# rust-cv/cv

Measured on AMD Instinct MI355X. Metric: frames/sec AKAZE detect+describe+BF-Hamming-match, 1080p, higher is better.
Workload: dtype f32; 1 GPU; BASELINE configs[1]: batch of 256 synthetic 1920x1080 frames per GPU (ONE panning camera over a single seeded world canvas, 4 px right / 2 px down per frame, +-2 sensor noise per frame — not SURVEY 8d's per-frame seeds: consecutive frames must overlap for the match to mean something), Akaze::default() detect+describe, + symmetric better-by-24 BF Hamming match of consecutive frames; micro_batch=256, parallelism=frame-sharded x1

## Files before the change

### cv_amd/_lib.py

```python
import ctypes as C
import os

import numpy as np

_HERE = os.path.dirname(os.path.abspath(__file__))
LIB_PATH = os.path.join(_HERE, "lib", "libakz.so")


class AkzError(RuntimeError):
    def __init__(self, status, what=""):
        self.status = status
        msg = lib().akz_strerror(status).decode()
        hip = lib().akz_last_hip_error()
        if status == -5 and hip:
            msg += f" (hip {hip}: {lib().akz_last_hip_error_string().decode()})"
        super().__init__(f"{what}: {msg}" if what else msg)


class Config(C.Structure):
    _fields_ = [
        ("maximum_features", C.c_uint64),
        ("num_sublevels", C.c_uint32),
        ("max_octave_evolution", C.c_uint32),
        ("base_scale_offset", C.c_double),
# ... 6 lines not shown
        ("descriptor_pattern_size", C.c_uint64),
    ]


class Options(C.Structure):
    _fields_ = [
        ("struct_size", C.c_uint32), ("flags", C.c_uint32), ("fed_block", C.c_uint32),
        ("sup_capacity", C.c_uint32), ("max_candidates", C.c_uint32), ("desc_tile_shift", C.c_uint32),
        ("stream_waves", C.c_uint32), ("stream_min_waves", C.c_uint32), ("arith", C.c_uint32), ("cu_ss", C.c_uint32),
        ("cu_kp", C.c_uint32), ("resident_min_frames", C.c_uint32), ("reserved", C.c_uint32 * 4),
    ]


OPT_KEEP_ALL, OPT_NO_FRAME_PAIRS, OPT_SERIAL_SUPPRESSION, OPT_NO_PIPELINE = 1, 2, 4, 8
OPT_STREAM_PRIORITY, OPT_CONTRAST_EXACT, OPT_CONTRAST_FORCE_ODD, OPT_TILE_KERNELS, OPT_SERIAL_DET, OPT_SPLIT_FRONT_FED, OPT_EQUAL_PRIORITY, OPT_NO_RESIDENT_LEVELS = 16, 32, 64, 128, 256, 512, 1024, 2048
HM_OPT_NO_FP4, HM_OPT_NO_MFMA, HM_OPT_STREAM_PRIORITY, HM_OPT_NO_LDS_DMA = 1, 2, 4, 8
FMT_U8, FMT_F32, FMT_U16 = 0, 1, 2
ARITH_REDUCE_PAIRWISE, ARITH_FMA, ARITH_HALF_SEQUENTIAL = 1, 2, 4


BOOL_OPTIONS = ("keep_all", "frame_pairs", "parallel_suppression", "pipeline", "stream_priority", "stream_kernels",
                "det_side_stream", "fuse_front_fed", "resident_levels")


def make_options(keep_all=False, frame_pairs=True, parallel_suppression=True, pipeline=True, stream_priority=True,
                 contrast="fine", fed_block=0, sup_capacity=0, max_candidates=0, desc_tile_shift=0, stream_kernels=True,
                 stream_waves=0, stream_min_waves=0, det_side_stream=True, fuse_front_fed=True, arith=0, cu_ss=0, cu_kp=0,
                 resident_levels=True, resident_min_frames=0):
    o = Options()
    o.struct_size = C.sizeof(Options)
    o.flags = ((OPT_KEEP_ALL if keep_all else 0) | (0 if frame_pairs else OPT_NO_FRAME_PAIRS)
               | (0 if parallel_suppression else OPT_SERIAL_SUPPRESSION) | (0 if pipeline else OPT_NO_PIPELINE)
               | (0 if stream_priority else OPT_EQUAL_PRIORITY) | (0 if stream_kernels else OPT_TILE_KERNELS)
               | (0 if det_side_stream else OPT_SERIAL_DET) | (0 if fuse_front_fed else OPT_SPLIT_FRONT_FED)
               | (0 if resident_levels else OPT_NO_RESIDENT_LEVELS)
               | {"fine": 0, "exact": OPT_CONTRAST_EXACT, "force_odd": OPT_CONTRAST_FORCE_ODD}[contrast])
    o.fed_block, o.sup_capacity, o.max_candidates, o.desc_tile_shift = fed_block, sup_capacity, max_candidates, desc_tile_shift
    o.stream_waves, o.stream_min_waves = stream_waves, stream_min_waves
    o.arith = arith
    o.cu_ss, o.cu_kp = cu_ss, cu_kp
    o.resident_min_frames = resident_min_frames
    return o


class ArrsacParams(C.Structure):
    _fields_ = [("struct_size", C.c_uint32), ("n_hypotheses", C.c_uint32), ("block_size", C.c_uint32),
                ("init_blocks", C.c_uint32), ("max_candidates", C.c_uint32), ("flags", C.c_uint32),
                ("threshold", C.c_double), ("sprt_delta", C.c_double), ("sprt_ratio", C.c_double), ("seed", C.c_uint64),
                ("estimations_per_block", C.c_uint32), ("reserved", C.c_uint32)]

# ... 210 lines not shown
```

### cv_amd/csrc/akz_api.hip

```cpp
#include <math.h>
#include <stdio.h>

#include <new>

#include "akz_ctx.h"

thread_local int g_akz_last_hip = 0;

extern "C" const char* akz_version(void) { return "cv_amd-akz 0.5 (gfx950)"; }
extern "C" uint32_t akz_abi_version(void) { return AKZ_ABI_VERSION; }

extern "C" const char* akz_strerror(int32_t s)
{
    switch (s) {
    case AKZ_OK: return "ok";
    case AKZ_E_INVALID: return "invalid argument or unsupported configuration";
    case AKZ_E_NO_DEVICE: return "no usable HIP device";
    case AKZ_E_OOM: return "out of device memory";
    case AKZ_E_CAPACITY: return "output buffer too small";
    case AKZ_E_HIP: return "HIP runtime error";
    case AKZ_E_TOO_LARGE: return "image or batch larger than the context was created for";
    case AKZ_E_INTERNAL: return "device-side overflow of an internal work list (create the context with a larger max_keypoints / akz_options.max_candidates)";
    case AKZ_E_COMM: return "RCCL call failed or librccl.so.1 could not be loaded (akz_comm_last_error_string())";
    default: return "unknown status";
// ... 117 lines not shown
{
    return akz_guard([&]() -> int32_t {
        if (!cfg || !out || max_w < 3 || max_h < 3 || max_batch < 1 || max_w > 65535 || max_h > 65535) return AKZ_E_INVALID;
        if ((size_t)max_w * (size_t)max_h > kAkzMaxPixels) return AKZ_E_TOO_LARGE;
        AKZ_TRY(validate_config(cfg));
        akz_options o;
        memset(&o, 0, sizeof(o));
        if (opts) {
            if (opts->struct_size < 2 * sizeof(uint32_t) || opts->struct_size > 4096) return AKZ_E_INVALID;
            memcpy(&o, opts, opts->struct_size < sizeof(o) ? opts->struct_size : sizeof(o));
            for (uint32_t i = (uint32_t)sizeof(o); i < opts->struct_size; ++i)
                if (reinterpret_cast<const unsigned char*>(opts)[i]) return AKZ_E_INVALID;
            if (o.cu_ss > 32 || o.cu_kp > 32) return AKZ_E_INVALID;
            for (uint32_t r : o.reserved)
                if (r) return AKZ_E_INVALID;
            if (o.flags & ~((AKZ_OPT_NO_RESIDENT_LEVELS << 1) - 1u)) return AKZ_E_INVALID;
            if (o.fed_block > 8 || (o.desc_tile_shift != 0 && (o.desc_tile_shift < 2 || o.desc_tile_shift > 9))) return AKZ_E_INVALID;
            if (o.arith > 7u) return AKZ_E_INVALID;
            if (o.sup_capacity > (1u << 24) || o.max_candidates > kAkzMaxKeypoints || o.stream_waves > (1u << 24) ||
                o.stream_min_waves > (1u << 24))
                return AKZ_E_INVALID;
        }
        {
            AkzPlan probe;
            akz_build_plan(*cfg, max_w, max_h, &probe);
            if ((int)probe.levels.size() > kAkzMaxLevels) return AKZ_E_INVALID;
        }
        int ndev = 0;
        hipError_t e = hipGetDeviceCount(&ndev);
        if (e != hipSuccess || ndev <= 0 || device < 0 || device >= ndev) {
            g_akz_last_hip = (int)e;
// ... 11 lines not shown
        c->max_w = max_w;
        c->max_h = max_h;
        c->max_batch = max_batch;
        c->max_kp = max_keypoints ? max_keypoints : 16384u;
        if (c->max_kp > kAkzMaxKeypoints) c->max_kp = kAkzMaxKeypoints;
        c->max_cand = o.max_candidates ? o.max_candidates : c->max_kp;
        if (c->max_cand > kAkzMaxKeypoints) c->max_cand = kAkzMaxKeypoints;
        c->sup_cap = o.sup_capacity ? o.sup_capacity : 4u * c->max_kp;
        c->sup_parallel = !(o.flags & AKZ_OPT_SERIAL_SUPPRESSION);
        c->keep_all = (o.flags & AKZ_OPT_KEEP_ALL) != 0;
        c->front_pair = !(o.flags & AKZ_OPT_NO_FRAME_PAIRS);
        c->stream_kernels = !(o.flags & AKZ_OPT_TILE_KERNELS);
        c->det_side_stream = !(o.flags & AKZ_OPT_SERIAL_DET);
        c->fuse_front_fed = !(o.flags & AKZ_OPT_SPLIT_FRONT_FED);
        c->resident_levels = !(o.flags & AKZ_OPT_NO_RESIDENT_LEVELS);
        c->resident_min_frames = (int)o.resident_min_frames;
        c->arith = (int)o.arith;
        if (o.stream_waves) c->det_stream_waves = (int)o.stream_waves;
        if (o.stream_min_waves) c->stream_min_waves = (size_t)o.stream_min_waves;
        c->contrast_fine = !(o.flags & AKZ_OPT_CONTRAST_EXACT);
        c->contrast_force_odd = (o.flags & AKZ_OPT_CONTRAST_FORCE_ODD) != 0;
        c->nsets = (o.flags & AKZ_OPT_NO_PIPELINE) ? 1 : 2;
        if (o.fed_block) c->fed_block = (int)o.fed_block;
        if (o.desc_tile_shift) c->desc_tile_shift = (int)o.desc_tile_shift;
        int32_t st = AKZ_OK;
        int prio_lo = 0, prio_hi = 0;
        hipDeviceGetStreamPriorityRange(&prio_lo, &prio_hi);
        const bool use_prio = !(o.flags & AKZ_OPT_EQUAL_PRIORITY);
        if (o.cu_ss) {
            if (akz_stream_on_cus(&c->stream, 0, (int)o.cu_ss) != hipSuccess) st = AKZ_E_HIP;
// ... 710 lines not shown
```

### cv_amd/csrc/akz_ctx.h

```cpp
#pragma once
#include <utility>

#include <hip/hip_ext.h>

#include "akz_common.h"

typedef akz_keypoint DevKp;

struct AkzTimer {
    std::vector<std::pair<hipEvent_t, hipEvent_t>> pending;
    std::vector<hipEvent_t> pool;
    hipEvent_t cur_start = nullptr;
    double ms = 0.0;
    uint64_t launches = 0, units = 0, units2 = 0;
};

struct AkzSet {
    std::vector<float*> Lt, Lsm, Ldet, Lflow;
    std::vector<float2*> Lxy;
    float* tmp = nullptr;
    void* d_in = nullptr;
    unsigned long long* d_cmax = nullptr;
    uint32_t* d_hist = nullptr;
    uint32_t* d_npoints = nullptr;
// ... 55 lines not shown

    AkzPlan plan;
    int cur_w = 0, cur_h = 0, cur_n = 0;

    void* arena = nullptr;
    size_t arena_bytes = 0;
    AkzSet sets[2];
    int nsets = 2;
    int cur = 0;
    uint64_t calls = 0;
    hipStream_t stream_kp = nullptr;
    hipStream_t stream_det = nullptr;
    bool det_side_stream = true;
    bool fuse_front_fed = true;
    bool resident_levels = true;
    int resident_min_frames = 0;
    hipEvent_t ev_level[kAkzMaxLevels] = {};
    hipEvent_t ev_det_done = nullptr;
    bool sup_parallel = true;
    uint32_t sup_cap = 0;
    void* d_color = nullptr;
    size_t color_bytes = 0;
    hipEvent_t ev_ss_done[2] = {nullptr, nullptr};
    hipEvent_t ev_kp_done[2] = {nullptr, nullptr};
    bool kp_pending[2] = {false, false};
    hipEvent_t ev_input = nullptr;
    AkzSet& S() { return sets[cur]; }
    void* h_in = nullptr;
    size_t h_in_bytes = 0;
    void* h_out = nullptr;
// ... 55 lines not shown
```

### cv_amd/csrc/akz_scale_space.hip

```cpp
#include "akz_ctx.h"

#ifndef AKZ_ARITH
#define AKZ_ARITH 0
#endif
#define AKZ_SS_CAT2(a, b) a##b
#define AKZ_SS_CAT(a, b) AKZ_SS_CAT2(a, b)
#define AKZ_SS(name) AKZ_SS_CAT(name##_arith, AKZ_ARITH)

namespace {

constexpr bool kArithPairwise = (AKZ_ARITH & 1) != 0;
constexpr bool kArithFma = (AKZ_ARITH & 2) != 0;
constexpr bool kArithHalfSeq = (AKZ_ARITH & 4) != 0;

constexpr int kTW = 64;
constexpr int kTH = 32;
constexpr int kDTH = 12;

enum { EPI_BLUR = 0, EPI_FLOW = 1, EPI_CMAX = 2, EPI_CHIST = 3 };

__device__ __forceinline__ int clampi(int v, int lo, int hi) { return v < lo ? lo : (v > hi ? hi : v); }

__device__ __forceinline__ uint3 xcd_tile_linear(uint32_t orig, uint3 grid);
__device__ __forceinline__ uint3 xcd_tile(uint3 bid, uint3 grid)
// ... 1019 lines not shown
    float v = l0;
    if (x < w - 1) v = v + fed_flow(half_tau, c0, C[1], l0, L[1]);
    if (x > 0) v = v - fed_flow(half_tau, C[-1], c0, L[-1], l0);
    if (y < h - 1) v = v + fed_flow(half_tau, c0, C[w], l0, L[w]);
    if (y > 0) v = v - fed_flow(half_tau, C[-w], c0, L[-w], l0);
    dst[base] = v;
}

constexpr int kFedMaxBlock = 16;
struct FedTaus {
    float half_tau[kFedMaxBlock];
};

constexpr int fed_halo_patches(int T) { return (T + 3) / 4; }
constexpr int fed_tile_edge(int T) { return 64 - 8 * fed_halo_patches(T); }

__device__ __forceinline__ v2f fed_flow2(v2f ht, v2f ca, v2f cb, v2f a, v2f b) { return (ht * (ca + cb)) * (b - a); }

__device__ __forceinline__ void fed_steps(v2f (&L)[4][4], v2f (&C)[4][4], float4* __restrict__ s_top,
                                          float4* __restrict__ s_ct, float4* __restrict__ s_vd, const FedTaus& taus,
                                          int nsteps, int tid, int up, int dn, int x0, int y0, int w, int h)
{
    s_ct[tid * 2] = make_float4(C[0][0].x, C[0][0].y, C[0][1].x, C[0][1].y);
    s_ct[tid * 2 + 1] = make_float4(C[0][2].x, C[0][2].y, C[0][3].x, C[0][3].y);
    const bool z_right = x0 + 4 <= 0 || x0 + 4 >= w;
    bool z_below[4];
#pragma unroll
    for (int r = 0; r < 4; ++r) z_below[r] = y0 + r < 0 || y0 + r >= h - 1;
#pragma unroll 1
    for (int t = 0; t < nsteps; ++t) {
// ... 33 lines not shown
                for (int c = 0; c < 4; ++c) vu[c] = fed_flow2(htu, C[r - (r > 0)][c], C[r][c], L[r - (r > 0)][c], L[r][c]);
            } else {
                __syncthreads();
                const float4 a = s_vd[up * 2], b = s_vd[up * 2 + 1];
                vu[0] = (v2f){a.x, a.y}; vu[1] = (v2f){a.z, a.w}; vu[2] = (v2f){b.x, b.y}; vu[3] = (v2f){b.z, b.w};
            }
#pragma unroll
            for (int c = 0; c < 4; ++c) {
                L[r][c] = (((L[r][c] + hf[c + 1]) - hf[c]) + vd[c]) - vu[c];
                vd[c] = vu[c];
            }
        }
    }
}

__device__ __forceinline__ void fed_steps_sums(v2f (&L)[4][4], const v2f (&C)[4][4], float4* __restrict__ s_top,
                                               float4* __restrict__ s_ct, float4* __restrict__ s_vd, const FedTaus& taus,
                                               int nsteps, int tid, int up, int dn, int x0, int y0, int w, int h)
{
    s_ct[tid * 2] = make_float4(C[0][0].x, C[0][0].y, C[0][1].x, C[0][1].y);
    s_ct[tid * 2 + 1] = make_float4(C[0][2].x, C[0][2].y, C[0][3].x, C[0][3].y);
    v2f SH[4][4], SV[4][4];
#pragma unroll
    for (int r = 0; r < 4; ++r) {
        const v2f Cr = dpp_row<0x101>(C[r][0]);
#pragma unroll
        for (int c = 0; c < 3; ++c) SH[r][c] = C[r][c] + C[r][c + 1];
        SH[r][3] = C[r][3] + Cr;
    }
#pragma unroll
    for (int r = 0; r < 3; ++r)
#pragma unroll
        for (int c = 0; c < 4; ++c) SV[r][c] = C[r][c] + C[r + 1][c];
    __syncthreads();
    {
        const float4 c = s_ct[dn * 2], d = s_ct[dn * 2 + 1];
        SV[3][0] = C[3][0] + (v2f){c.x, c.y};
        SV[3][1] = C[3][1] + (v2f){c.z, c.w};
        SV[3][2] = C[3][2] + (v2f){d.x, d.y};
        SV[3][3] = C[3][3] + (v2f){d.z, d.w};
    }
    const bool z_right = x0 + 4 <= 0 || x0 + 4 >= w;
    bool z_below[4];
#pragma unroll
    for (int r = 0; r < 4; ++r) z_below[r] = y0 + r < 0 || y0 + r >= h - 1;
#pragma unroll 1
    for (int t = 0; t < nsteps; ++t) {
        const float htf = taus.half_tau[t];
        const v2f ht = splat(htf);
        s_top[tid * 2] = make_float4(L[0][0].x, L[0][0].y, L[0][1].x, L[0][1].y);
        s_top[tid * 2 + 1] = make_float4(L[0][2].x, L[0][2].y, L[0][3].x, L[0][3].y);
        __syncthreads();
        v2f vd[4];
        {
            const float4 a = s_top[dn * 2], b = s_top[dn * 2 + 1];
            const v2f Lb[4] = {(v2f){a.x, a.y}, (v2f){a.z, a.w}, (v2f){b.x, b.y}, (v2f){b.z, b.w}};
            const v2f ht3 = splat(z_below[3] ? 0.0f : htf);
#pragma unroll
            for (int cc = 0; cc < 4; ++cc) vd[cc] = (ht3 * SV[3][cc]) * (Lb[cc] - L[3][cc]);
            s_vd[tid * 2] = make_float4(vd[0].x, vd[0].y, vd[1].x, vd[1].y);
            s_vd[tid * 2 + 1] = make_float4(vd[2].x, vd[2].y, vd[3].x, vd[3].y);
        }
        const v2f htr = splat(z_right ? 0.0f : htf);
#pragma unroll
        for (int r = 3; r >= 0; --r) {
            const v2f Lr = dpp_row<0x101>(L[r][0]);
            v2f hf[5];
#pragma unroll
            for (int c = 1; c < 4; ++c) hf[c] = (ht * SH[r][c - 1]) * (L[r][c] - L[r][c - 1]);
            hf[4] = (htr * SH[r][3]) * (Lr - L[r][3]);
            hf[0] = dpp_row<0x111>(hf[4]);
            v2f vu[4];
            if (r > 0) {
                const v2f htu = splat(z_below[r > 0 ? r - 1 : 0] ? 0.0f : htf);
#pragma unroll
                for (int c = 0; c < 4; ++c) vu[c] = (htu * SV[r - (r > 0)][c]) * (L[r][c] - L[r - (r > 0)][c]);
            } else {
                __syncthreads();
                const float4 a = s_vd[up * 2], b = s_vd[up * 2 + 1];
                vu[0] = (v2f){a.x, a.y}; vu[1] = (v2f){a.z, a.w}; vu[2] = (v2f){b.x, b.y}; vu[3] = (v2f){b.z, b.w};
            }
#pragma unroll
            for (int c = 0; c < 4; ++c) {
                L[r][c] = (((L[r][c] + hf[c + 1]) - hf[c]) + vd[c]) - vu[c];
                vd[c] = vu[c];
            }
        }
    }
}

__device__ __forceinline__ void fed_store_patch(const v2f (&L)[4][4], float* __restrict__ dst, int fa, int fb, bool has_b,
                                                size_t fs, int w, int h, int x0, int y0)
{
    float* da = dst + (size_t)fa * fs;
    float* db = dst + (size_t)fb * fs;
// ... 101 lines not shown
                                                const float* __restrict__ srcb, int w, int wx0, int wy0, int tid)
{
    constexpr int NCH = kFFIn * (kFFInC / 4);
#pragma unroll
    for (int i = 0; i < ITEMS; ++i) {
        const int idx = tid + 256 * i;
        if (idx < NCH) {
            const int iy = idx / (kFFInC / 4), c4 = idx - iy * (kFFInC / 4);
            const uint32_t o = (uint32_t)((wy0 - 3 + iy) * w + (wx0 - 4 + 4 * c4)) << 2;
            ra[i] = *reinterpret_cast<const float4*>(at_bytes(srca, o));
            rb[i] = *reinterpret_cast<const float4*>(at_bytes(srcb, o));
        }
    }
}

template <int SG, int HP, bool RING, bool WRITE_FLOW>
__global__ __launch_bounds__(256, kFFWaves) void k_front_fed(const float* __restrict__ in, int w, int h, size_t fs, int n,
                                                      GaussTaps taps, OffK k, FedTaus taus, int nsteps,
                                                      float* __restrict__ out_lt, float* __restrict__ out_flow,
                                                      float2* __restrict__ out_xy, const float* __restrict__ invk,
                                                      int invk_off, float* __restrict__ half_out, size_t half_fs)
{
    __shared__ __attribute__((aligned(16))) v2f s_buf[kFFIn * kFFInC];
    static_assert((kFFW + 2) * kFFGS <= kFFIn * kFFInC, "blurred window fits in the input window's space");
    static_assert(3 * 256 * 2 * 2 <= kFFIn * kFFInC, "FED exchange buffers fit");
    constexpr int U = front_fed_tile(HP);
    const uint3 tile = xcd_tile(make_uint3(blockIdx.x, blockIdx.y, blockIdx.z), make_uint3(gridDim.x, gridDim.y, gridDim.z));
    const int tid = threadIdx.x, pc = tid & 15, pr = tid >> 4;
    const int fa = 2 * (int)tile.z;
    const bool has_b = fa + 1 < n;
    const int fb = has_b ? fa + 1 : fa;
    const int wx0 = (int)tile.x * U - 4 * HP, wy0 = (int)tile.y * U - 4 * HP;
    const float* srca = in + (size_t)fa * fs;
    const float* srcb = in + (size_t)fb * fs;
    {
        const bool inside = wx0 >= 4 && wx0 + kFFW + 4 <= w && wy0 >= 3 && wy0 + kFFW + 3 <= h;
        if (inside) {
            constexpr int NCH = kFFIn * (kFFInC / 4), ITEMS = (NCH + 255) / 256;
            float4 ra[ITEMS], rb[ITEMS];
            front_fed_fetch<ITEMS>(ra, rb, srca, srcb, w, wx0, wy0, tid);
            float4* d = reinterpret_cast<float4*>(s_buf);
#pragma unroll
            for (int i = 0; i < ITEMS; ++i) {
                const int idx = tid + 256 * i;
                if (idx < NCH) {
                    const int iy = idx / (kFFInC / 4), c4 = idx - iy * (kFFInC / 4);
                    d[ff_chunk<kFFInC / 2>(iy, 2 * c4)] = make_float4(ra[i].x, rb[i].x, ra[i].y, rb[i].y);
                    d[ff_chunk<kFFInC / 2>(iy, 2 * c4 + 1)] = make_float4(ra[i].z, rb[i].z, ra[i].w, rb[i].w);
                }
            }
        } else {
            constexpr int NE = kFFIn * kFFInC, BATCH = 8;
            for (int base = 0; base < NE; base += 256 * BATCH) {
                float ea[BATCH], eb[BATCH];
#pragma unroll
                for (int i = 0; i < BATCH; ++i) {
                    const int idx = base + tid + 256 * i;
                    ea[i] = eb[i] = 0.0f;
                    if (idx < NE) {
                        const int iy = idx / kFFInC, ix = idx - iy * kFFInC;
                        const int cx = clampi(wx0 - 4 + ix, 0, w - 1), cy = clampi(wy0 - 3 + iy, 0, h - 1);
                        const size_t o = (size_t)cy * w + cx;
                        ea[i] = srca[o];
                        eb[i] = srcb[o];
                    }
                }
#pragma unroll
                for (int i = 0; i < BATCH; ++i) {
                    const int idx = base + tid + 256 * i;
                    if (idx < NE) {
                        const int iy = idx / kFFInC, ix = idx - iy * kFFInC;
                        s_buf[ff_elem<kFFInC / 2>(iy, ix)] = (v2f){ea[i], eb[i]};
                    }
                }
            }
        }
    }
    __syncthreads();
    v2f g[4][4];
// ... 73 lines not shown
            }
        }
#pragma unroll
        for (int j = 0; j < 4; ++j)
#pragma unroll
            for (int o = 0; o < 4; ++o) {
                const v2f col[5] = {hb[j][o], hb[j + 1][o], hb[j + 2][o], hb[j + 3][o], hb[j + 4][o]};
                g[j][o] = lane4_dot_v<5>(col, taps.k);
            }
    }
    __syncthreads();
    v2f* s_g = s_buf;
    float4* g4 = reinterpret_cast<float4*>(s_buf);
#pragma unroll
    for (int j = 0; j < 4; ++j) {
        g4[ff_chunk<kFFGS / 2>(4 * pr + j + 1, 2 * pc + 1)] = make_float4(g[j][0].x, g[j][0].y, g[j][1].x, g[j][1].y);
        g4[ff_chunk<kFFGS / 2>(4 * pr + j + 1, 2 * pc + 2)] = make_float4(g[j][2].x, g[j][2].y, g[j][3].x, g[j][3].y);
    }
#pragma unroll
    for (int q = 0; q < 2; ++q)
        if (RING && tid + 256 * q < 4 * kFFW + 4) s_g[ff_elem<kFFGS / 2>(ring_y[q] + 1, ring_x[q] + 2)] = ring[q];
    __syncthreads();
    if (wx0 < 1 || wx0 + kFFW + 1 > w || wy0 < 1 || wy0 + kFFW + 1 > h) {
#pragma unroll
        for (int j = 0; j < 4; ++j)
#pragma unroll
            for (int o = 0; o < 4; ++o) {
                const int x = wx0 + 4 * pc + o, y = wy0 + 4 * pr + j;
                const int xc = clampi(x, 0, w - 1), yc = clampi(y, 0, h - 1);
                if (xc != x || yc != y) {
                    const int X = clampi(xc - wx0, -1, kFFW), Y = clampi(yc - wy0, -1, kFFW);
                    s_g[ff_elem<kFFGS / 2>(4 * pr + j + 1, 4 * pc + o + 2)] = s_g[ff_elem<kFFGS / 2>(Y + 1, X + 2)];
                }
            }
#pragma unroll
        for (int q = 0; q < 2; ++q)
            if (RING && tid + 256 * q < 4 * kFFW + 4) {
                const int x = wx0 + ring_x[q], y = wy0 + ring_y[q];
                const int xc = clampi(x, 0, w - 1), yc = clampi(y, 0, h - 1);
                if (xc != x || yc != y) {
                    const int X = clampi(xc - wx0, -1, kFFW), Y = clampi(yc - wy0, -1, kFFW);
                    s_g[ff_elem<kFFGS / 2>(ring_y[q] + 1, ring_x[q] + 2)] = s_g[ff_elem<kFFGS / 2>(Y + 1, X + 2)];
                }
            }
        __syncthreads();
    }
    const int x0 = wx0 + 4 * pc, y0 = wy0 + 4 * pr;
    const bool col_in = x0 >= 0 && x0 < w;
    const bool useful = pc >= HP && pc <= 15 - HP && pr >= HP && pr <= 15 - HP && col_in;
    v2f C[4][4];
    {
        const v2f inverse_k = (v2f){invk[(size_t)fa * 8 + invk_off], invk[(size_t)fb * 8 + invk_off]};
        v2f hx[3][4], hy[3][4];
#pragma unroll
        for (int r = 0; r < 6; ++r) {
            v2f v[8];
#pragma unroll
            for (int q = 0; q < 4; ++q) {
                const f4v t = lds_chunk(g4 + ff_chunk<kFFGS / 2>(4 * pr + r, 2 * pc + q));
                v[2 * q] = (v2f){t.x, t.y};
                v[2 * q + 1] = (v2f){t.z, t.w};
            }
            const int s = r % 3;
#pragma unroll
            for (int o = 0; o < 4; ++o) {
                hx[s][o] = v[o + 3] - v[o + 1];
                hy[s][o] = (splat(3.0f) * v[o + 1] + splat(10.0f) * v[o + 2]) + splat(3.0f) * v[o + 3];
            }
            if (r >= 2) {
                const int j = r - 2, sm = (r - 2) % 3, s0 = (r - 1) % 3, sp = r % 3;
                v2f den[4];
#pragma unroll
                for (int o = 0; o < 4; ++o) {
                    const v2f lx = (splat(3.0f) * hx[sm][o] + splat(10.0f) * hx[s0][o]) + splat(3.0f) * hx[sp][o];
// ... 6 lines not shown
#pragma unroll
                    for (int o = 0; o < 4; ++o) C[j][o] = splat(1.0f) / den[o];
                } else {
#pragma unroll
                    for (int o = 0; o < 4; ++o) C[j][o] = rcp_pair_finite(den[o]);
                }
            }
        }
    }
    if (WRITE_FLOW && useful) {
#pragma unroll
        for (int j = 0; j < 4; ++j) {
            const int y = y0 + j;
            if (y >= h) break;
            const uint32_t o = (uint32_t)(y * w + x0) << 2;
            *reinterpret_cast<float4*>(at_bytes(out_flow + (size_t)fa * fs, o)) = make_float4(C[j][0].x, C[j][1].x, C[j][2].x, C[j][3].x);
            if (has_b)
                *reinterpret_cast<float4*>(at_bytes(out_flow + (size_t)fb * fs, o)) = make_float4(C[j][0].y, C[j][1].y, C[j][2].y, C[j][3].y);
        }
    }
    if (useful) {
#pragma unroll
        for (int j = 0; j < 4; ++j) {
            const int y = y0 + j;
            if (y >= h) break;
            v2f m[12], z[12], p[12];
            const int Y = 4 * pr + j;
            constexpr int Q0 = (4 - SG) / 2, Q1 = (7 + SG) / 2;
#pragma unroll
            for (int q = Q0; q <= Q1; ++q) {
                const f4v a = lds_chunk(g4 + ff_chunk<kFFGS / 2>(Y - SG + 1, 2 * pc - 1 + q));
                const f4v b = lds_chunk(g4 + ff_chunk<kFFGS / 2>(Y + 1, 2 * pc - 1 + q));
                const f4v c = lds_chunk(g4 + ff_chunk<kFFGS / 2>(Y + SG + 1, 2 * pc - 1 + q));
                m[2 * q] = (v2f){a.x, a.y}; m[2 * q + 1] = (v2f){a.z, a.w};
                z[2 * q] = (v2f){b.x, b.y}; z[2 * q + 1] = (v2f){b.z, b.w};
                p[2 * q] = (v2f){c.x, c.y}; p[2 * q + 1] = (v2f){c.z, c.w};
            }
            v2f rx[4], ry[4];
#pragma unroll
            for (int o = 0; o < 4; ++o) {
                const v2f mm = m[4 + o - SG], m0 = m[4 + o], mp = m[4 + o + SG];
                const v2f zm = z[4 + o - SG], zp = z[4 + o + SG];
                const v2f pm = p[4 + o - SG], p0 = p[4 + o], pp = p[4 + o + SG];
                rx[o] = off_combine_sg<SG>(k, mp - mm, zp - zm, pp - pm);
                ry[o] = off_combine_sg<SG>(k, pm, p0, pp) - off_combine_sg<SG>(k, mm, m0, mp);
            }
            const uint32_t o = (uint32_t)(y * w + x0) << 3;
            {
                float4* xy = reinterpret_cast<float4*>(at_bytes(out_xy + (size_t)fa * fs, o));
                xy[0] = make_float4(rx[0].x, ry[0].x, rx[1].x, ry[1].x);
                xy[1] = make_float4(rx[2].x, ry[2].x, rx[3].x, ry[3].x);
            }
            if (has_b) {
                float4* xy = reinterpret_cast<float4*>(at_bytes(out_xy + (size_t)fb * fs, o));
                xy[0] = make_float4(rx[0].y, ry[0].y, rx[1].y, ry[1].y);
                xy[1] = make_float4(rx[2].y, ry[2].y, rx[3].y, ry[3].y);
            }
        }
    }
#pragma unroll
    for (int r = 0; r < 4; ++r) {
        const int y = y0 + r;
        const bool in_img = col_in && y >= 0 && y < h;
        if (!in_img) {
#pragma unroll
            for (int c = 0; c < 4; ++c) {
                L[r][c] = splat(0.0f);
                C[r][c] = splat(0.0f);
            }
        }
    }
    __syncthreads();
    float4* s_top = reinterpret_cast<float4*>(s_buf);
    float4* s_vd = s_top + 256 * 2;
    float4* s_ct = s_vd + 256 * 2;
    const int up = pr > 0 ? tid - 16 : tid, dn = pr < 15 ? tid + 16 : tid;
    fed_steps_sums(L, C, s_top, s_ct, s_vd, taus, nsteps, tid, up, dn, x0, y0, w, h);
    if (useful) {
        fed_store_patch(L, out_lt, fa, fb, has_b, fs, w, h, x0, y0);
        if (half_out) fed_store_half(L, half_out, fa, fb, has_b, half_fs, w, h, x0, y0);
    }
}

constexpr int kResMaxSteps = 64;
struct FedTausN {
    float half_tau[kResMaxSteps];
};
constexpr int kResLdsBytes = 160 * 1024 - 2048;
#ifndef AKZ_RES_R
#define AKZ_RES_R 6
#define AKZ_RES_WAVES 12
#endif

__device__ __forceinline__ int res_chunk(int rs, int row, int ci) { return row * rs + ((ci & 1) ? (rs >> 1) : 0) + (ci >> 1); }
__device__ __forceinline__ int res_elem(int rs, int row, int col) { return 2 * res_chunk(rs, row, col >> 1) + (col & 1); }
// ... 1212 lines not shown
                    int ngr = (left + fed_block - 1) / fed_block;
                    int g = (left + ngr - 1) / ngr;
                    groups.push_back(g);
                    left -= g;
                }
            const bool front_fed = c->fuse_front_fed && blocked && fused_front && !c->keep_all && !groups.empty() &&
                                   groups[0] <= (L.octave == 0 ? 4 : 8);
            if (front_fed) {
                const int ng = (int)groups.size();
                float* dst0 = ((ng - 1) % 2 == 0) ? bufA : bufB;
                FedTaus ft;
                for (int q = 0; q < kFedMaxBlock; ++q) ft.half_tau[q] = q < groups[0] ? 0.5f * (float)L.tau[q] : 0.0f;
                OffK kk = make_offk(L.deriv_sigma);
                const int t_ff = (L.octave == 0 ? AKZ_T_FRONT_FED_SG2 : AKZ_T_FRONT_FED_DEEP_SG2) + (int)L.deriv_sigma - 2;
                akz_timer_begin(c, t_ff, s);
#define AKZ_FF3(SGV, HPV, RGV, WFV)                                                                                  \
    AKZ_LAUNCH((k_front_fed<SGV, HPV, RGV, WFV>),                                                             \
                       dim3(akz_div_up(L.w, front_fed_tile(HPV)), akz_div_up(L.h, front_fed_tile(HPV)), (n + 1) / 2), \
                       dim3(256), 0, s, init, L.w, L.h, fs, n, t1, kk, ft, groups[0], dst0, S.Lflow[i], S.Lxy[i],      \
                       (const float*)S.d_invk, (int)L.octave, ng == 1 ? half_next : (float*)nullptr, half_next_fs)
#define AKZ_FF2(SGV, HPV, RGV) if (ng > 1) { AKZ_FF3(SGV, HPV, RGV, true); } else { AKZ_FF3(SGV, HPV, RGV, false); }
#define AKZ_FF(SGV)                                                                                                  \
    if (groups[0] <= 3) { AKZ_FF2(SGV, 1, false) } else if (groups[0] == 4) { AKZ_FF2(SGV, 1, true) }               \
    else if (groups[0] <= 7) { AKZ_FF2(SGV, 2, false) } else { AKZ_FF2(SGV, 2, true) }
                switch (L.deriv_sigma) {
                case 2: AKZ_FF(2) break;
                case 3: AKZ_FF(3) break;
                default: AKZ_FF(4) break;
                }
#undef AKZ_FF
#undef AKZ_FF2
#undef AKZ_FF3
                AKZ_LAUNCH_CHECK();
                akz_timer_end(c, t_ff, s, 1, (uint64_t)fs * n);
            } else if (fused_front) {
                akz_timer_begin(c, t_front, s);
                float* lsm_out = c->keep_all ? S.Lsm[i] : nullptr;
                dim3 gridf(akz_div_up(L.w, kTW), akz_div_up(L.h, kTH), n);
                OffK kk = make_offk(L.deriv_sigma);
#define AKZ_FRONT(SGV)                                                                                               \
    AKZ_LAUNCH((k_level_front<2, SGV, float, true>), gridf, dim3(256), 0, s, init, L.w, L.h, fs, t1, kk,      \
                       lsm_out, S.Lflow[i], S.Lxy[i], (const float*)S.d_invk, (int)L.octave)
#define AKZ_FRONT2X(SGV, THV, NTV, TPBV)                                                                             \
    AKZ_LAUNCH((k_level_front2<2, SGV, THV, NTV, float, true, TPBV>),                                            \
                       dim3(akz_div_up(L.w, kTW), akz_div_up(akz_div_up(L.h, THV), TPBV), (n + 1) / 2), dim3(NTV), 0, s, \
                       init, L.w, L.h, fs, n, t1, kk, lsm_out, S.Lflow[i], S.Lxy[i], (const float*)S.d_invk,            \
                       (int)L.octave)
// ... 166 lines not shown
```

### include/akz.h

```cpp
#ifndef AKZ_H
#define AKZ_H

#include <stdint.h>

#ifdef __cplusplus
extern "C" {
#endif

typedef enum akz_status {
    AKZ_OK = 0,
    AKZ_E_INVALID = -1,
    AKZ_E_NO_DEVICE = -2,
    AKZ_E_OOM = -3,
    AKZ_E_CAPACITY = -4,
    AKZ_E_HIP = -5,
    AKZ_E_TOO_LARGE = -6,
    AKZ_E_INTERNAL = -7,
    AKZ_E_COMM = -8
} akz_status;

typedef struct akz_config {
    uint64_t maximum_features;
    uint32_t num_sublevels;
    uint32_t max_octave_evolution;
// ... 35 lines not shown
                   int32_t max_batch, uint32_t max_keypoints, akz_ctx** out);
int32_t akz_destroy(akz_ctx* ctx);

enum {
    AKZ_OPT_KEEP_ALL = 1u << 0,
    AKZ_OPT_NO_FRAME_PAIRS = 1u << 1,
    AKZ_OPT_SERIAL_SUPPRESSION = 1u << 2,
    AKZ_OPT_NO_PIPELINE = 1u << 3,
    AKZ_OPT_STREAM_PRIORITY = 1u << 4,
    AKZ_OPT_CONTRAST_EXACT = 1u << 5,
    AKZ_OPT_CONTRAST_FORCE_ODD = 1u << 6,
    AKZ_OPT_TILE_KERNELS = 1u << 7,
    AKZ_OPT_SERIAL_DET = 1u << 8,
    AKZ_OPT_SPLIT_FRONT_FED = 1u << 9,
    AKZ_OPT_EQUAL_PRIORITY = 1u << 10,
    AKZ_OPT_NO_RESIDENT_LEVELS = 1u << 11
};
typedef struct akz_options {
    uint32_t struct_size;
    uint32_t flags;
    uint32_t fed_block;
    uint32_t sup_capacity;
    uint32_t max_candidates;
    uint32_t desc_tile_shift;
    uint32_t stream_waves;
    uint32_t stream_min_waves;
    uint32_t arith;
    uint32_t cu_ss;
    uint32_t cu_kp;
    uint32_t resident_min_frames;
    uint32_t reserved[4];
// ... 292 lines not shown
```

Before: 9242 frames/s.

## Pack two vertically adjacent halves of one frame into front-FED v2f lanes

```diff
diff --git a/cv_amd/_lib.py b/cv_amd/_lib.py
--- a/cv_amd/_lib.py
+++ b/cv_amd/_lib.py
@@ -44,26 +44,27 @@
 
 OPT_KEEP_ALL, OPT_NO_FRAME_PAIRS, OPT_SERIAL_SUPPRESSION, OPT_NO_PIPELINE = 1, 2, 4, 8
 OPT_STREAM_PRIORITY, OPT_CONTRAST_EXACT, OPT_CONTRAST_FORCE_ODD, OPT_TILE_KERNELS, OPT_SERIAL_DET, OPT_SPLIT_FRONT_FED, OPT_EQUAL_PRIORITY, OPT_NO_RESIDENT_LEVELS = 16, 32, 64, 128, 256, 512, 1024, 2048
+OPT_NO_HALF_WINDOWS = 4096
 HM_OPT_NO_FP4, HM_OPT_NO_MFMA, HM_OPT_STREAM_PRIORITY, HM_OPT_NO_LDS_DMA = 1, 2, 4, 8
 FMT_U8, FMT_F32, FMT_U16 = 0, 1, 2
 ARITH_REDUCE_PAIRWISE, ARITH_FMA, ARITH_HALF_SEQUENTIAL = 1, 2, 4
 
 
 BOOL_OPTIONS = ("keep_all", "frame_pairs", "parallel_suppression", "pipeline", "stream_priority", "stream_kernels",
-                "det_side_stream", "fuse_front_fed", "resident_levels")
+                "det_side_stream", "fuse_front_fed", "resident_levels", "half_windows")
 
 
 def make_options(keep_all=False, frame_pairs=True, parallel_suppression=True, pipeline=True, stream_priority=True,
                  contrast="fine", fed_block=0, sup_capacity=0, max_candidates=0, desc_tile_shift=0, stream_kernels=True,
                  stream_waves=0, stream_min_waves=0, det_side_stream=True, fuse_front_fed=True, arith=0, cu_ss=0, cu_kp=0,
-                 resident_levels=True, resident_min_frames=0):
+                 resident_levels=True, resident_min_frames=0, half_windows=True):
     o = Options()
     o.struct_size = C.sizeof(Options)
     o.flags = ((OPT_KEEP_ALL if keep_all else 0) | (0 if frame_pairs else OPT_NO_FRAME_PAIRS)
                | (0 if parallel_suppression else OPT_SERIAL_SUPPRESSION) | (0 if pipeline else OPT_NO_PIPELINE)
                | (0 if stream_priority else OPT_EQUAL_PRIORITY) | (0 if stream_kernels else OPT_TILE_KERNELS)
                | (0 if det_side_stream else OPT_SERIAL_DET) | (0 if fuse_front_fed else OPT_SPLIT_FRONT_FED)
-               | (0 if resident_levels else OPT_NO_RESIDENT_LEVELS)
+               | (0 if resident_levels else OPT_NO_RESIDENT_LEVELS) | (0 if half_windows else OPT_NO_HALF_WINDOWS)
                | {"fine": 0, "exact": OPT_CONTRAST_EXACT, "force_odd": OPT_CONTRAST_FORCE_ODD}[contrast])
     o.fed_block, o.sup_capacity, o.max_candidates, o.desc_tile_shift = fed_block, sup_capacity, max_candidates, desc_tile_shift
     o.stream_waves, o.stream_min_waves = stream_waves, stream_min_waves
diff --git a/cv_amd/csrc/akz_api.hip b/cv_amd/csrc/akz_api.hip
--- a/cv_amd/csrc/akz_api.hip
+++ b/cv_amd/csrc/akz_api.hip
@@ -155,7 +155,7 @@
             if (o.cu_ss > 32 || o.cu_kp > 32) return AKZ_E_INVALID;
             for (uint32_t r : o.reserved)
                 if (r) return AKZ_E_INVALID;
-            if (o.flags & ~((AKZ_OPT_NO_RESIDENT_LEVELS << 1) - 1u)) return AKZ_E_INVALID;
+            if (o.flags & ~((AKZ_OPT_NO_HALF_WINDOWS << 1) - 1u)) return AKZ_E_INVALID;
             if (o.fed_block > 8 || (o.desc_tile_shift != 0 && (o.desc_tile_shift < 2 || o.desc_tile_shift > 9))) return AKZ_E_INVALID;
             if (o.arith > 7u) return AKZ_E_INVALID;
             if (o.sup_capacity > (1u << 24) || o.max_candidates > kAkzMaxKeypoints || o.stream_waves > (1u << 24) ||
@@ -197,6 +197,7 @@
         c->det_side_stream = !(o.flags & AKZ_OPT_SERIAL_DET);
         c->fuse_front_fed = !(o.flags & AKZ_OPT_SPLIT_FRONT_FED);
         c->resident_levels = !(o.flags & AKZ_OPT_NO_RESIDENT_LEVELS);
+        c->half_windows = !(o.flags & AKZ_OPT_NO_HALF_WINDOWS);
         c->resident_min_frames = (int)o.resident_min_frames;
         c->arith = (int)o.arith;
         if (o.stream_waves) c->det_stream_waves = (int)o.stream_waves;
diff --git a/cv_amd/csrc/akz_ctx.h b/cv_amd/csrc/akz_ctx.h
--- a/cv_amd/csrc/akz_ctx.h
+++ b/cv_amd/csrc/akz_ctx.h
@@ -93,6 +93,7 @@
     bool det_side_stream = true;
     bool fuse_front_fed = true;
     bool resident_levels = true;
+    bool half_windows = true;
     int resident_min_frames = 0;
     hipEvent_t ev_level[kAkzMaxLevels] = {};
     hipEvent_t ev_det_done = nullptr;
diff --git a/cv_amd/csrc/akz_scale_space.hip b/cv_amd/csrc/akz_scale_space.hip
--- a/cv_amd/csrc/akz_scale_space.hip
+++ b/cv_amd/csrc/akz_scale_space.hip
@@ -1057,6 +1057,7 @@
 
 constexpr int fed_halo_patches(int T) { return (T + 3) / 4; }
 constexpr int fed_tile_edge(int T) { return 64 - 8 * fed_halo_patches(T); }
+constexpr int kSeamRows = 64;
 
 __device__ __forceinline__ v2f fed_flow2(v2f ht, v2f ca, v2f cb, v2f a, v2f b) { return (ht * (ca + cb)) * (b - a); }
 
@@ -1120,9 +1121,11 @@
     }
 }
 
+template <bool SEAM = false>
 __device__ __forceinline__ void fed_steps_sums(v2f (&L)[4][4], const v2f (&C)[4][4], float4* __restrict__ s_top,
                                                float4* __restrict__ s_ct, float4* __restrict__ s_vd, const FedTaus& taus,
-                                               int nsteps, int tid, int up, int dn, int x0, int y0, int w, int h)
+                                               int nsteps, int tid, int up, int dn, int x0, int y0, int w, int h,
+                                               bool seam_dn = false, bool seam_up = false)
 {
     s_ct[tid * 2] = make_float4(C[0][0].x, C[0][0].y, C[0][1].x, C[0][1].y);
     s_ct[tid * 2 + 1] = make_float4(C[0][2].x, C[0][2].y, C[0][3].x, C[0][3].y);
@@ -1141,27 +1144,41 @@
     __syncthreads();
     {
         const float4 c = s_ct[dn * 2], d = s_ct[dn * 2 + 1];
-        SV[3][0] = C[3][0] + (v2f){c.x, c.y};
-        SV[3][1] = C[3][1] + (v2f){c.z, c.w};
-        SV[3][2] = C[3][2] + (v2f){d.x, d.y};
-        SV[3][3] = C[3][3] + (v2f){d.z, d.w};
+        v2f Cb[4] = {(v2f){c.x, c.y}, (v2f){c.z, c.w}, (v2f){d.x, d.y}, (v2f){d.z, d.w}};
+        if (SEAM && seam_dn) {
+#pragma unroll
+            for (int cc = 0; cc < 4; ++cc) Cb[cc] = splat(Cb[cc].y);
+        }
+#pragma unroll
+        for (int cc = 0; cc < 4; ++cc) SV[3][cc] = C[3][cc] + Cb[cc];
     }
     const bool z_right = x0 + 4 <= 0 || x0 + 4 >= w;
-    bool z_below[4];
-#pragma unroll
-    for (int r = 0; r < 4; ++r) z_below[r] = y0 + r < 0 || y0 + r >= h - 1;
+    bool z_below[4], z_below_b[4];
+#pragma unroll
+    for (int r = 0; r < 4; ++r) {
+        z_below[r] = y0 + r < 0 || y0 + r >= h - 1;
+        z_below_b[r] = y0 + kSeamRows + r >= h - 1;
+    }
 #pragma unroll 1
     for (int t = 0; t < nsteps; ++t) {
         const float htf = taus.half_tau[t];
         const v2f ht = splat(htf);
+        auto ht_row = [&](int r) -> v2f {
+            if constexpr (SEAM) return (v2f){z_below[r] ? 0.0f : htf, z_below_b[r] ? 0.0f : htf};
+            else return splat(z_below[r] ? 0.0f : htf);
+        };
         s_top[tid * 2] = make_float4(L[0][0].x, L[0][0].y, L[0][1].x, L[0][1].y);
         s_top[tid * 2 + 1] = make_float4(L[0][2].x, L[0][2].y, L[0][3].x, L[0][3].y);
         __syncthreads();
         v2f vd[4];
         {
             const float4 a = s_top[dn * 2], b = s_top[dn * 2 + 1];
-            const v2f Lb[4] = {(v2f){a.x, a.y}, (v2f){a.z, a.w}, (v2f){b.x, b.y}, (v2f){b.z, b.w}};
-            const v2f ht3 = splat(z_below[3] ? 0.0f : htf);
+            v2f Lb[4] = {(v2f){a.x, a.y}, (v2f){a.z, a.w}, (v2f){b.x, b.y}, (v2f){b.z, b.w}};
+            if (SEAM && seam_dn) {
+#pragma unroll
+                for (int cc = 0; cc < 4; ++cc) Lb[cc] = splat(Lb[cc].y);
+            }
+            const v2f ht3 = ht_row(3);
 #pragma unroll
             for (int cc = 0; cc < 4; ++cc) vd[cc] = (ht3 * SV[3][cc]) * (Lb[cc] - L[3][cc]);
             s_vd[tid * 2] = make_float4(vd[0].x, vd[0].y, vd[1].x, vd[1].y);
@@ -1178,13 +1195,17 @@
             hf[0] = dpp_row<0x111>(hf[4]);
             v2f vu[4];
             if (r > 0) {
-                const v2f htu = splat(z_below[r > 0 ? r - 1 : 0] ? 0.0f : htf);
+                const v2f htu = ht_row(r > 0 ? r - 1 : 0);
 #pragma unroll
                 for (int c = 0; c < 4; ++c) vu[c] = (htu * SV[r - (r > 0)][c]) * (L[r][c] - L[r - (r > 0)][c]);
             } else {
                 __syncthreads();
                 const float4 a = s_vd[up * 2], b = s_vd[up * 2 + 1];
                 vu[0] = (v2f){a.x, a.y}; vu[1] = (v2f){a.z, a.w}; vu[2] = (v2f){b.x, b.y}; vu[3] = (v2f){b.z, b.w};
+                if (SEAM && seam_up) {
+#pragma unroll
+                    for (int c = 0; c < 4; ++c) vu[c] = (v2f){0.0f, vu[c].x};
+                }
             }
 #pragma unroll
             for (int c = 0; c < 4; ++c) {
@@ -1316,7 +1337,24 @@
     }
 }
 
-template <int SG, int HP, bool RING, bool WRITE_FLOW>
+template <int ITEMS>
+__device__ __forceinline__ void front_fed_fetch_halves(float4 (&ra)[ITEMS], float4 (&rb)[ITEMS], const float* __restrict__ src,
+                                                       int w, int h, int wx0, int wy0, int tid)
+{
+    constexpr int NCH = kFFIn * (kFFInC / 4);
+#pragma unroll
+    for (int i = 0; i < ITEMS; ++i) {
+        const int idx = tid + 256 * i;
+        if (idx < NCH) {
+            const int iy = idx / (kFFInC / 4), c4 = idx - iy * (kFFInC / 4);
+            const int ya = clampi(wy0 - 3 + iy, 0, h - 1), yb = clampi(wy0 + kSeamRows - 3 + iy, 0, h - 1);
+            ra[i] = *reinterpret_cast<const float4*>(at_bytes(src, (uint32_t)(ya * w + (wx0 - 4 + 4 * c4)) << 2));
+            rb[i] = *reinterpret_cast<const float4*>(at_bytes(src, (uint32_t)(yb * w + (wx0 - 4 + 4 * c4)) << 2));
+        }
+    }
+}
+
+template <int SG, int HP, bool RING, bool WRITE_FLOW, bool HALVES = false>
 __global__ __launch_bounds__(256, kFFWaves) void k_front_fed(const float* __restrict__ in, int w, int h, size_t fs, int n,
                                                       GaussTaps taps, OffK k, FedTaus taus, int nsteps,
                                                       float* __restrict__ out_lt, float* __restrict__ out_flow,
@@ -1324,23 +1362,26 @@
                                                       int invk_off, float* __restrict__ half_out, size_t half_fs)
 {
     __shared__ __attribute__((aligned(16))) v2f s_buf[kFFIn * kFFInC];
-    static_assert((kFFW + 2) * kFFGS <= kFFIn * kFFInC, "blurred window fits in the input window's space");
+    constexpr int GA = HALVES ? 4 : 1;
+    static_assert((kFFW + 2 * GA) * kFFGS <= kFFIn * kFFInC, "blurred window fits in the input window's space");
     static_assert(3 * 256 * 2 * 2 <= kFFIn * kFFInC, "FED exchange buffers fit");
     constexpr int U = front_fed_tile(HP);
     const uint3 tile = xcd_tile(make_uint3(blockIdx.x, blockIdx.y, blockIdx.z), make_uint3(gridDim.x, gridDim.y, gridDim.z));
     const int tid = threadIdx.x, pc = tid & 15, pr = tid >> 4;
-    const int fa = 2 * (int)tile.z;
-    const bool has_b = fa + 1 < n;
+    const int fa = HALVES ? (int)tile.z : 2 * (int)tile.z;
+    const bool has_b = !HALVES && fa + 1 < n;
     const int fb = has_b ? fa + 1 : fa;
-    const int wx0 = (int)tile.x * U - 4 * HP, wy0 = (int)tile.y * U - 4 * HP;
+    constexpr int YB = HALVES ? kSeamRows : 0;
+    const int wx0 = (int)tile.x * U - 4 * HP, wy0 = (int)tile.y * (U + YB) - 4 * HP;
     const float* srca = in + (size_t)fa * fs;
     const float* srcb = in + (size_t)fb * fs;
     {
-        const bool inside = wx0 >= 4 && wx0 + kFFW + 4 <= w && wy0 >= 3 && wy0 + kFFW + 3 <= h;
+        const bool inside = wx0 >= 4 && wx0 + kFFW + 4 <= w && (HALVES || (wy0 >= 3 && wy0 + kFFW + 3 <= h));
         if (inside) {
             constexpr int NCH = kFFIn * (kFFInC / 4), ITEMS = (NCH + 255) / 256;
             float4 ra[ITEMS], rb[ITEMS];
-            front_fed_fetch<ITEMS>(ra, rb, srca, srcb, w, wx0, wy0, tid);
+            if constexpr (HALVES) front_fed_fetch_halves<ITEMS>(ra, rb, srca, w, h, wx0, wy0, tid);
+            else front_fed_fetch<ITEMS>(ra, rb, srca, srcb, w, wx0, wy0, tid);
             float4* d = reinterpret_cast<float4*>(s_buf);
 #pragma unroll
             for (int i = 0; i < ITEMS; ++i) {
@@ -1364,7 +1405,7 @@
                         const int cx = clampi(wx0 - 4 + ix, 0, w - 1), cy = clampi(wy0 - 3 + iy, 0, h - 1);
                         const size_t o = (size_t)cy * w + cx;
                         ea[i] = srca[o];
-                        eb[i] = srcb[o];
+                        eb[i] = HALVES ? srca[(size_t)clampi(wy0 + YB - 3 + iy, 0, h - 1) * w + cx] : srcb[o];
                     }
                 }
 #pragma unroll
@@ -1468,13 +1509,14 @@
     float4* g4 = reinterpret_cast<float4*>(s_buf);
 #pragma unroll
     for (int j = 0; j < 4; ++j) {
-        g4[ff_chunk<kFFGS / 2>(4 * pr + j + 1, 2 * pc + 1)] = make_float4(g[j][0].x, g[j][0].y, g[j][1].x, g[j][1].y);
-        g4[ff_chunk<kFFGS / 2>(4 * pr + j + 1, 2 * pc + 2)] = make_float4(g[j][2].x, g[j][2].y, g[j][3].x, g[j][3].y);
+        g4[ff_chunk<kFFGS / 2>(4 * pr + j + GA, 2 * pc + 1)] = make_float4(g[j][0].x, g[j][0].y, g[j][1].x, g[j][1].y);
+        g4[ff_chunk<kFFGS / 2>(4 * pr + j + GA, 2 * pc + 2)] = make_float4(g[j][2].x, g[j][2].y, g[j][3].x, g[j][3].y);
     }
 #pragma unroll
     for (int q = 0; q < 2; ++q)
-        if (RING && tid + 256 * q < 4 * kFFW + 4) s_g[ff_elem<kFFGS / 2>(ring_y[q] + 1, ring_x[q] + 2)] = ring[q];
+        if (RING && tid + 256 * q < 4 * kFFW + 4) s_g[ff_elem<kFFGS / 2>(ring_y[q] + GA, ring_x[q] + 2)] = ring[q];
     __syncthreads();
+    if constexpr (!HALVES) {
     if (wx0 < 1 || wx0 + kFFW + 1 > w || wy0 < 1 || wy0 + kFFW + 1 > h) {
 #pragma unroll
         for (int j = 0; j < 4; ++j)
@@ -1499,9 +1541,51 @@
             }
         __syncthreads();
     }
+    } else {
+        float* s_gf = reinterpret_cast<float*>(s_buf);
+        constexpr int SW = kFFW + 2, NSEAM = 4 * SW;
+        int seam_x[2], seam_r[2];
+#pragma unroll
+        for (int q = 0; q < 2; ++q) {
+            const int t = tid + 256 * q;
+            seam_r[q] = t / SW;
+            seam_x[q] = t - seam_r[q] * SW - 1;
+            if (t < NSEAM) {
+                s_gf[2 * ff_elem<kFFGS / 2>(kFFW + seam_r[q] + GA, seam_x[q] + 2)] = s_gf[2 * ff_elem<kFFGS / 2>(seam_r[q] + GA, seam_x[q] + 2) + 1];
+                s_gf[2 * ff_elem<kFFGS / 2>(seam_r[q] - 4 + GA, seam_x[q] + 2) + 1] = s_gf[2 * ff_elem<kFFGS / 2>(kFFW - 4 + seam_r[q] + GA, seam_x[q] + 2)];
+            }
+        }
+        __syncthreads();
+        if (wx0 < 1 || wx0 + kFFW + 1 > w || wy0 < 1 || wy0 + YB + kFFW + 1 > h) {
+#pragma unroll
+            for (int f = 0; f < 2; ++f) {
+                const int wyf = wy0 + f * YB, Y0 = f ? -4 : -1, Y1 = f ? kFFW : kFFW + 3;
+                auto fix = [&](int X, int Y) {
+                    const int x = wx0 + X, y = wyf + Y;
+                    const int xc = clampi(x, 0, w - 1), yc = clampi(y, 0, h - 1);
+                    if (xc != x || yc != y) {
+                        const int Xs = clampi(xc - wx0, -1, kFFW), Ys = clampi(yc - wyf, Y0, Y1);
+                        s_gf[2 * ff_elem<kFFGS / 2>(Y + GA, X + 2) + f] = s_gf[2 * ff_elem<kFFGS / 2>(Ys + GA, Xs + 2) + f];
+                    }
+                };
+#pragma unroll
+                for (int j = 0; j < 4; ++j)
+#pragma unroll
+                    for (int o = 0; o < 4; ++o) fix(4 * pc + o, 4 * pr + j);
+#pragma unroll
+                for (int q = 0; q < 2; ++q) {
+                    if (RING && tid + 256 * q < 4 * kFFW + 4 && ring_y[q] != (f ? -1 : kFFW)) fix(ring_x[q], ring_y[q]);
+                    if (tid + 256 * q < NSEAM) fix(seam_x[q], f ? seam_r[q] - 4 : kFFW + seam_r[q]);
+                }
+            }
+            __syncthreads();
+        }
+    }
     const int x0 = wx0 + 4 * pc, y0 = wy0 + 4 * pr;
     const bool col_in = x0 >= 0 && x0 < w;
-    const bool useful = pc >= HP && pc <= 15 - HP && pr >= HP && pr <= 15 - HP && col_in;
+    const bool useful_a = pc >= HP && pc <= 15 - HP && pr >= HP && (HALVES || pr <= 15 - HP) && col_in;
+    const bool useful_b = pc >= HP && pc <= 15 - HP && (HALVES || pr >= HP) && pr <= 15 - HP && col_in;
+    const bool useful = useful_a || useful_b;
     v2f C[4][4];
     {
         const v2f inverse_k = (v2f){invk[(size_t)fa * 8 + invk_off], invk[(size_t)fb * 8 + invk_off]};
@@ -1511,7 +1595,7 @@
             v2f v[8];
 #pragma unroll
             for (int q = 0; q < 4; ++q) {
-                const f4v t = lds_chunk(g4 + ff_chunk<kFFGS / 2>(4 * pr + r, 2 * pc + q));
+                const f4v t = lds_chunk(g4 + ff_chunk<kFFGS / 2>(4 * pr + r - 1 + GA, 2 * pc + q));
                 v[2 * q] = (v2f){t.x, t.y};
                 v[2 * q + 1] = (v2f){t.z, t.w};
             }
@@ -1548,9 +1632,10 @@
             const int y = y0 + j;
             if (y >= h) break;
             const uint32_t o = (uint32_t)(y * w + x0) << 2;
-            *reinterpret_cast<float4*>(at_bytes(out_flow + (size_t)fa * fs, o)) = make_float4(C[j][0].x, C[j][1].x, C[j][2].x, C[j][3].x);
-            if (has_b)
-                *reinterpret_cast<float4*>(at_bytes(out_flow + (size_t)fb * fs, o)) = make_float4(C[j][0].y, C[j][1].y, C[j][2].y, C[j][3].y);
+            if (!HALVES || useful_a)
+                *reinterpret_cast<float4*>(at_bytes(out_flow + (size_t)fa * fs, o)) = make_float4(C[j][0].x, C[j][1].x, C[j][2].x, C[j][3].x);
+            if (HALVES ? useful_b && y + YB < h : has_b)
+                *reinterpret_cast<float4*>(at_bytes(out_flow + (size_t)fb * fs, o + ((uint32_t)(YB * w) << 2))) = make_float4(C[j][0].y, C[j][1].y, C[j][2].y, C[j][3].y);
         }
     }
     if (useful) {
@@ -1563,9 +1648,9 @@
             constexpr int Q0 = (4 - SG) / 2, Q1 = (7 + SG) / 2;
 #pragma unroll
             for (int q = Q0; q <= Q1; ++q) {
-                const f4v a = lds_chunk(g4 + ff_chunk<kFFGS / 2>(Y - SG + 1, 2 * pc - 1 + q));
-                const f4v b = lds_chunk(g4 + ff_chunk<kFFGS / 2>(Y + 1, 2 * pc - 1 + q));
-                const f4v c = lds_chunk(g4 + ff_chunk<kFFGS / 2>(Y + SG + 1, 2 * pc - 1 + q));
+                const f4v a = lds_chunk(g4 + ff_chunk<kFFGS / 2>(Y - SG + GA, 2 * pc - 1 + q));
+                const f4v b = lds_chunk(g4 + ff_chunk<kFFGS / 2>(Y + GA, 2 * pc - 1 + q));
+                const f4v c = lds_chunk(g4 + ff_chunk<kFFGS / 2>(Y + SG + GA, 2 * pc - 1 + q));
                 m[2 * q] = (v2f){a.x, a.y}; m[2 * q + 1] = (v2f){a.z, a.w};
                 z[2 * q] = (v2f){b.x, b.y}; z[2 * q + 1] = (v2f){b.z, b.w};
                 p[2 * q] = (v2f){c.x, c.y}; p[2 * q + 1] = (v2f){c.z, c.w};
@@ -1580,13 +1665,13 @@
                 ry[o] = off_combine_sg<SG>(k, pm, p0, pp) - off_combine_sg<SG>(k, mm, m0, mp);
             }
             const uint32_t o = (uint32_t)(y * w + x0) << 3;
-            {
+            if (!HALVES || useful_a) {
                 float4* xy = reinterpret_cast<float4*>(at_bytes(out_xy + (size_t)fa * fs, o));
                 xy[0] = make_float4(rx[0].x, ry[0].x, rx[1].x, ry[1].x);
                 xy[1] = make_float4(rx[2].x, ry[2].x, rx[3].x, ry[3].x);
             }
-            if (has_b) {
-                float4* xy = reinterpret_cast<float4*>(at_bytes(out_xy + (size_t)fb * fs, o));
+            if (HALVES ? useful_b && y + YB < h : has_b) {
+                float4* xy = reinterpret_cast<float4*>(at_bytes(out_xy + (size_t)fb * fs, o + ((uint32_t)(YB * w) << 3)));
                 xy[0] = make_float4(rx[0].y, ry[0].y, rx[1].y, ry[1].y);
                 xy[1] = make_float4(rx[2].y, ry[2].y, rx[3].y, ry[3].y);
             }
@@ -1596,11 +1681,24 @@
     for (int r = 0; r < 4; ++r) {
         const int y = y0 + r;
         const bool in_img = col_in && y >= 0 && y < h;
-        if (!in_img) {
+        const bool in_img_b = HALVES ? col_in && y + YB < h : in_img;
+        if (!in_img && !in_img_b) {
 #pragma unroll
             for (int c = 0; c < 4; ++c) {
                 L[r][c] = splat(0.0f);
                 C[r][c] = splat(0.0f);
+            }
+        } else if (HALVES && !in_img) {
+#pragma unroll
+            for (int c = 0; c < 4; ++c) {
+                L[r][c] = (v2f){0.0f, L[r][c].y};
+                C[r][c] = (v2f){0.0f, C[r][c].y};
+            }
+        } else if (HALVES && !in_img_b) {
+#pragma unroll
+            for (int c = 0; c < 4; ++c) {
+                L[r][c] = (v2f){L[r][c].x, 0.0f};
+                C[r][c] = (v2f){C[r][c].x, 0.0f};
             }
         }
     }
@@ -1608,11 +1706,29 @@
     float4* s_top = reinterpret_cast<float4*>(s_buf);
     float4* s_vd = s_top + 256 * 2;
     float4* s_ct = s_vd + 256 * 2;
-    const int up = pr > 0 ? tid - 16 : tid, dn = pr < 15 ? tid + 16 : tid;
-    fed_steps_sums(L, C, s_top, s_ct, s_vd, taus, nsteps, tid, up, dn, x0, y0, w, h);
-    if (useful) {
-        fed_store_patch(L, out_lt, fa, fb, has_b, fs, w, h, x0, y0);
-        if (half_out) fed_store_half(L, half_out, fa, fb, has_b, half_fs, w, h, x0, y0);
+    if constexpr (!HALVES) {
+        const int up = pr > 0 ? tid - 16 : tid, dn = pr < 15 ? tid + 16 : tid;
+        fed_steps_sums(L, C, s_top, s_ct, s_vd, taus, nsteps, tid, up, dn, x0, y0, w, h);
+        if (useful) {
+            fed_store_patch(L, out_lt, fa, fb, has_b, fs, w, h, x0, y0);
+            if (half_out) fed_store_half(L, half_out, fa, fb, has_b, half_fs, w, h, x0, y0);
+        }
+    } else {
+        const int up = pr > 0 ? tid - 16 : tid + 240, dn = pr < 15 ? tid + 16 : tid - 240;
+        fed_steps_sums<true>(L, C, s_top, s_ct, s_vd, taus, nsteps, tid, up, dn, x0, y0, w, h, pr == 15, pr == 0);
+        if (useful_a) {
+            fed_store_patch(L, out_lt, fa, fa, false, fs, w, h, x0, y0);
+            if (half_out) fed_store_half(L, half_out, fa, fa, false, half_fs, w, h, x0, y0);
+        }
+        if (useful_b) {
+            v2f Lb[4][4];
+#pragma unroll
+            for (int r = 0; r < 4; ++r)
+#pragma unroll
+                for (int c = 0; c < 4; ++c) Lb[r][c] = splat(L[r][c].y);
+            fed_store_patch(Lb, out_lt, fa, fa, false, fs, w, h, x0, y0 + YB);
+            if (half_out) fed_store_half(Lb, half_out, fa, fa, false, half_fs, w, h, x0, y0 + YB);
+        }
     }
 }
 
@@ -2855,12 +2971,16 @@
                 OffK kk = make_offk(L.deriv_sigma);
                 const int t_ff = (L.octave == 0 ? AKZ_T_FRONT_FED_SG2 : AKZ_T_FRONT_FED_DEEP_SG2) + (int)L.deriv_sigma - 2;
                 akz_timer_begin(c, t_ff, s);
-#define AKZ_FF3(SGV, HPV, RGV, WFV)                                                                                  \
-    AKZ_LAUNCH((k_front_fed<SGV, HPV, RGV, WFV>),                                                             \
-                       dim3(akz_div_up(L.w, front_fed_tile(HPV)), akz_div_up(L.h, front_fed_tile(HPV)), (n + 1) / 2), \
+                const int ff_hp = groups[0] <= 4 ? 1 : 2;
+                const bool ff_halves = c->half_windows && akz_div_up(L.h, front_fed_tile(ff_hp)) > 1;
+#define AKZ_FF4(SGV, HPV, RGV, WFV, HVV)                                                                             \
+    AKZ_LAUNCH((k_front_fed<SGV, HPV, RGV, WFV, HVV>),                                                        \
+                       dim3(akz_div_up(L.w, front_fed_tile(HPV)),                                                       \
+                            akz_div_up(L.h, front_fed_tile(HPV) + (HVV ? kSeamRows : 0)), HVV ? n : (n + 1) / 2),      \
                        dim3(256), 0, s, init, L.w, L.h, fs, n, t1, kk, ft, groups[0], dst0, S.Lflow[i], S.Lxy[i],      \
                        (const float*)S.d_invk, (int)L.octave, ng == 1 ? half_next : (float*)nullptr, half_next_fs)
-#define AKZ_FF2(SGV, HPV, RGV) if (ng > 1) { AKZ_FF3(SGV, HPV, RGV, true); } else { AKZ_FF3(SGV, HPV, RGV, false); }
+#define AKZ_FF3(SGV, HPV, RGV, WFV) if (ff_halves) { AKZ_FF4(SGV, HPV, RGV, WFV, true); } else { AKZ_FF4(SGV, HPV, RGV, WFV, false); }
+#define AKZ_FF2(SGV, HPV, RGV) if (ng > 1) { AKZ_FF3(SGV, HPV, RGV, true) } else { AKZ_FF3(SGV, HPV, RGV, false) }
 #define AKZ_FF(SGV)                                                                                                  \
     if (groups[0] <= 3) { AKZ_FF2(SGV, 1, false) } else if (groups[0] == 4) { AKZ_FF2(SGV, 1, true) }               \
     else if (groups[0] <= 7) { AKZ_FF2(SGV, 2, false) } else { AKZ_FF2(SGV, 2, true) }
@@ -2872,6 +2992,7 @@
 #undef AKZ_FF
 #undef AKZ_FF2
 #undef AKZ_FF3
+#undef AKZ_FF4
                 AKZ_LAUNCH_CHECK();
                 akz_timer_end(c, t_ff, s, 1, (uint64_t)fs * n);
             } else if (fused_front) {
diff --git a/include/akz.h b/include/akz.h
--- a/include/akz.h
+++ b/include/akz.h
@@ -73,7 +73,8 @@
     AKZ_OPT_SERIAL_DET = 1u << 8,
     AKZ_OPT_SPLIT_FRONT_FED = 1u << 9,
     AKZ_OPT_EQUAL_PRIORITY = 1u << 10,
-    AKZ_OPT_NO_RESIDENT_LEVELS = 1u << 11
+    AKZ_OPT_NO_RESIDENT_LEVELS = 1u << 11,
+    AKZ_OPT_NO_HALF_WINDOWS = 1u << 12
 };
 typedef struct akz_options {
     uint32_t struct_size;
```

New measurement: 9291 frames/s, median of 6. No clear change (+0.5%).
